# nv-nguyen/gigapose

Hardware: NVIDIA H100
Metric: detections/sec (224x224 crops, 162-template bank) (higher is better)
Workload: dtype f32 (a1, a4, a6: bf16 hi/lo split x3 on tensor cores with fp32 accumulate = fp32-faithful; a5, a7-a9: fp32)

## Files before the change

gigapose_b200/csrc/common.cuh:

```cuda
#pragma once
#include <cuda_runtime.h>
#include <cuda.h>
#include <stdint.h>
#include <cstdio>

namespace gp {

__device__ __forceinline__ uint32_t smem_u32(const void* p) {
  return static_cast<uint32_t>(__cvta_generic_to_shared(p));
}

__device__ __forceinline__ bool elect_one() {
  uint32_t pred = 0;
  asm volatile(
      "{\n\t.reg .pred P;\n\t"
      "elect.sync _|P, 0xffffffff;\n\t"
      "selp.b32 %0, 1, 0, P;\n\t}"
      : "=r"(pred));
  return pred != 0;
}

__device__ __forceinline__ void mbar_init(uint64_t* bar, uint32_t count) {
  asm volatile("mbarrier.init.shared::cta.b64 [%0], %1;" ::"r"(smem_u32(bar)), "r"(count) : "memory");
}
__device__ __forceinline__ void fence_barrier_init() {
  asm volatile("fence.mbarrier_init.release.cluster;" ::: "memory");
}
__device__ __forceinline__ void fence_proxy_async() {
  asm volatile("fence.proxy.async.shared::cta;" ::: "memory");
}
__device__ __forceinline__ void mbar_arrive_expect_tx(uint64_t* bar, uint32_t bytes) {
  asm volatile("mbarrier.arrive.expect_tx.shared::cta.b64 _, [%0], %1;" ::"r"(smem_u32(bar)), "r"(bytes) : "memory");
}
__device__ __forceinline__ void mbar_arrive(uint64_t* bar) {
  asm volatile("mbarrier.arrive.shared::cta.b64 _, [%0];" ::"r"(smem_u32(bar)) : "memory");
}
__device__ __forceinline__ bool mbar_try_wait(uint64_t* bar, uint32_t parity) {
  uint32_t ok;
  asm volatile(
      "{\n\t.reg .pred P;\n\t"
      "mbarrier.try_wait.parity.shared::cta.b64 P, [%1], %2;\n\t"
      "selp.b32 %0, 1, 0, P;\n\t}"
      : "=r"(ok)
      : "r"(smem_u32(bar)), "r"(parity)
      : "memory");
  return ok != 0;
}
__device__ __forceinline__ void mbar_wait(uint64_t* bar, uint32_t parity) {
  uint32_t spins = 0;
  while (!mbar_try_wait(bar, parity)) {
    if (++spins > (1u << 26)) __trap();
  }
}

__device__ __forceinline__ void tma_prefetch_desc(const CUtensorMap* map) {
  asm volatile("prefetch.tensormap [%0];" ::"l"(reinterpret_cast<uint64_t>(map)) : "memory");
}
__device__ __forceinline__ void tma_load_2d(void* smem_dst, const CUtensorMap* map, uint64_t* bar, int32_t c0, int32_t c1) {
  asm volatile(
      "cp.async.bulk.tensor.2d.shared::cluster.global.mbarrier::complete_tx::bytes [%0], [%1, {%3, %4}], [%2];"
      ::"r"(smem_u32(smem_dst)), "l"(reinterpret_cast<uint64_t>(map)), "r"(smem_u32(bar)), "r"(c0), "r"(c1)
      : "memory");
}
__device__ __forceinline__ void tma_load_4d(void* smem_dst, const CUtensorMap* map, uint64_t* bar, int32_t c0, int32_t c1,
                                            int32_t c2, int32_t c3) {
  asm volatile(
      "cp.async.bulk.tensor.4d.shared::cluster.global.mbarrier::complete_tx::bytes [%0], [%1, {%3, %4, %5, %6}], [%2];"
      ::"r"(smem_u32(smem_dst)), "l"(reinterpret_cast<uint64_t>(map)), "r"(smem_u32(bar)), "r"(c0), "r"(c1), "r"(c2), "r"(c3)
      : "memory");
}
constexpr uint64_t kEvictFirst = 0x12F0000000000000ull;
constexpr uint64_t kEvictLast = 0x14F0000000000000ull;
__device__ __forceinline__ void tma_load_2d_hint(void* smem_dst, const CUtensorMap* map, uint64_t* bar, int32_t c0,
                                                 int32_t c1, uint64_t hint) {
  asm volatile(
      "cp.async.bulk.tensor.2d.shared::cluster.global.mbarrier::complete_tx::bytes.L2::cache_hint"
      " [%0], [%1, {%3, %4}], [%2], %5;"
      ::"r"(smem_u32(smem_dst)), "l"(reinterpret_cast<uint64_t>(map)), "r"(smem_u32(bar)), "r"(c0), "r"(c1), "l"(hint)
      : "memory");
}

template <int kRowBytes>
__device__ __forceinline__ uint64_t wgmma_desc_kmajor(uint32_t smem_addr) {
  static_assert(kRowBytes == 128 || kRowBytes == 64 || kRowBytes == 32, "swizzle span");
  constexpr uint64_t layout = kRowBytes == 128 ? 1 : (kRowBytes == 64 ? 2 : 3);
  constexpr uint64_t sbo = (8 * kRowBytes) >> 4;
  uint64_t d = 0;
  d |= static_cast<uint64_t>((smem_addr >> 4) & 0x3FFF);
  d |= 1ull << 16;
  d |= sbo << 32;
  d |= layout << 62;
  return d;
}

__device__ __forceinline__ uint64_t wgmma_desc_mnmajor_sw128(uint32_t smem_addr) {
  uint64_t d = 0;
  d |= static_cast<uint64_t>((smem_addr >> 4) & 0x3FFF);
  d |= 1ull << 16;
  d |= static_cast<uint64_t>(1024 >> 4) << 32;
  d |= 1ull << 62;
  return d;
}

__device__ __forceinline__ void pdl_trigger() { asm volatile("griddepcontrol.launch_dependents;" ::: "memory"); }
__device__ __forceinline__ void pdl_wait() { asm volatile("griddepcontrol.wait;" ::: "memory"); }

__device__ __forceinline__ void named_barrier_sync(uint32_t id, uint32_t nthreads) {
  asm volatile("bar.sync %0, %1;" ::"r"(id), "r"(nthreads) : "memory");
}

template <uint32_t kRegs>
__device__ __forceinline__ void setmaxnreg_dec() { asm volatile("setmaxnreg.dec.sync.aligned.u32 %0;" ::"n"(kRegs)); }
template <uint32_t kRegs>
__device__ __forceinline__ void setmaxnreg_inc() { asm volatile("setmaxnreg.inc.sync.aligned.u32 %0;" ::"n"(kRegs)); }

}
```

gigapose_b200/csrc/vit_attention_tc.cu:

```cuda
#include "gigapose_kernels.h"
#include "common.cuh"
#include "wgmma.cuh"
#include <cuda_bf16.h>

namespace gp {

namespace {

constexpr int kTok = 257, kDim = 1024, kHeads = 16, kHd = 64;
constexpr int kKeys = 272;
constexpr int kRow = 128;
constexpr int kKVPlane = kKeys * kRow;
constexpr int kQPlane = 256 * kRow;
constexpr int kQTiles = 4;
constexpr int kMmaWarps = 8;
constexpr int kThreads = (kMmaWarps + 1) * 32;

struct __align__(8) AttnTail {
  uint64_t qk_full, v_full;
};
constexpr int kSmem = 1024 + 4 * kKVPlane + 2 * kQPlane + sizeof(AttnTail);

__device__ __forceinline__ void split_pair(float a, float b, uint32_t& hi, uint32_t& lo) {
  asm("cvt.rn.bf16x2.f32 %0, %1, %2;" : "=r"(hi) : "f"(b), "f"(a));
  const float ra = a - __uint_as_float(hi << 16), rb = b - __uint_as_float(hi & 0xffff0000u);
  asm("cvt.rn.bf16x2.f32 %0, %1, %2;" : "=r"(lo) : "f"(rb), "f"(ra));
}
__device__ __forceinline__ float ex2_approx(float x) {
  float y;
  asm("ex2.approx.ftz.f32 %0, %1;" : "=f"(y) : "f"(x));
  return y;
}
constexpr float kExpScale = 0.125f * 1.4426950408889634f;
__device__ __forceinline__ float2 ld_pair_sw128(const uint8_t* hi, const uint8_t* lo, int row, int col) {
  const uint32_t off = (uint32_t)row * 128u + ((((uint32_t)col >> 3) ^ ((uint32_t)row & 7u)) << 4) + (((uint32_t)col & 7u) << 1);
  const uint32_t h = *reinterpret_cast<const uint32_t*>(hi + off);
  const uint32_t l = lo ? *reinterpret_cast<const uint32_t*>(lo + off) : 0u;
  return make_float2(__uint_as_float(h << 16) + __uint_as_float(l << 16),
                     __uint_as_float(h & 0xffff0000u) + __uint_as_float(l & 0xffff0000u));
}

}

__device__ long long g_attn_stamp[32];
#define STAMP(i) do { if (blockIdx.x == 0) g_attn_stamp[i] = clock64(); } while (0)

template <int kPasses>
__global__ void __launch_bounds__(kThreads, 1)
attention_tc_kernel(const __grid_constant__ CUtensorMap tm_hi_128, const __grid_constant__ CUtensorMap tm_lo_128,
                    const __grid_constant__ CUtensorMap tm_hi_16, const __grid_constant__ CUtensorMap tm_lo_16,
                    const __nv_bfloat16* __restrict__ qkv_hi, const __nv_bfloat16* __restrict__ qkv_lo,
                    __nv_bfloat16* __restrict__ out_hi, __nv_bfloat16* __restrict__ out_lo, int crop_stride) {
  constexpr int passes = kPasses;
  constexpr int np = passes == 3 ? 2 : 1;
  extern __shared__ uint8_t smem_raw[];
  pdl_trigger();
  uint8_t* smem = smem_raw + ((1024u - (smem_u32(smem_raw) & 1023u)) & 1023u);
  uint8_t* sK[2] = {smem, smem + kKVPlane};
  uint8_t* sV[2] = {smem + 2 * kKVPlane, smem + 3 * kKVPlane};
  uint8_t* sQ[2] = {smem + 4 * kKVPlane, smem + 4 * kKVPlane + kQPlane};
  AttnTail& tail = *reinterpret_cast<AttnTail*>(smem + 4 * kKVPlane + 2 * kQPlane);
  const int warp = threadIdx.x >> 5, lane = threadIdx.x & 31;
  const int item = blockIdx.x;
  const int img = item / kHeads, head = item % kHeads;
  const int row0 = img * kTok;
  const int rq = ((0 * crop_stride + img) * kHeads + head) * kTok;
  const int rk = ((1 * crop_stride + img) * kHeads + head) * kTok;
  const int rv = ((2 * crop_stride + img) * kHeads + head) * kTok;

  if (threadIdx.x == 0) {
    mbar_init(&tail.qk_full, 1);
    mbar_init(&tail.v_full, 1);
    fence_barrier_init();
  }
  __syncthreads();
  pdl_wait();
  if (threadIdx.x == 0) STAMP(0);

  if (warp == kMmaWarps) {
    if (lane == 0) {
      tma_prefetch_desc(&tm_hi_128); tma_prefetch_desc(&tm_hi_16);
      if (np == 2) { tma_prefetch_desc(&tm_lo_128); tma_prefetch_desc(&tm_lo_16); }
      mbar_arrive_expect_tx(&tail.qk_full, (uint32_t)(np * (kQPlane + kKVPlane)));
      for (int pl = 0; pl < np; ++pl) {
        const CUtensorMap* m128 = pl ? &tm_lo_128 : &tm_hi_128;
        const CUtensorMap* m16 = pl ? &tm_lo_16 : &tm_hi_16;
        tma_load_2d(sQ[pl], m128, &tail.qk_full, 0, rq);
        tma_load_2d(sQ[pl] + 128 * kRow, m128, &tail.qk_full, 0, rq + 128);
        tma_load_2d(sK[pl], m128, &tail.qk_full, 0, rk);
        tma_load_2d(sK[pl] + 128 * kRow, m128, &tail.qk_full, 0, rk + 128);
        tma_load_2d(sK[pl] + 256 * kRow, m16, &tail.qk_full, 0, rk + 256);
      }
      mbar_arrive_expect_tx(&tail.v_full, (uint32_t)(np * kKVPlane));
      for (int pl = 0; pl < np; ++pl) {
        const CUtensorMap* m128 = pl ? &tm_lo_128 : &tm_hi_128;
        const CUtensorMap* m16 = pl ? &tm_lo_16 : &tm_hi_16;
        tma_load_2d(sV[pl], m128, &tail.v_full, 0, rv);
        tma_load_2d(sV[pl] + 128 * kRow, m128, &tail.v_full, 0, rv + 128);
        tma_load_2d(sV[pl] + 256 * kRow, m16, &tail.v_full, 0, rv + 256);
      }
    }
    __syncwarp();
    __shared__ float s_p[kKeys];
    __shared__ float s_q[kHd];
    {
    const size_t qoff = (size_t)(rq + 256) * kHd + 2 * lane;
    const uint32_t qh = *reinterpret_cast<const uint32_t*>(qkv_hi + qoff);
    const uint32_t ql = passes == 3 ? *reinterpret_cast<const uint32_t*>(qkv_lo + qoff) : 0u;
    s_q[2 * lane] = __uint_as_float(qh << 16) + __uint_as_float(ql << 16);
    s_q[2 * lane + 1] = __uint_as_float(qh & 0xffff0000u) + __uint_as_float(ql & 0xffff0000u);
    __syncwarp();
    mbar_wait(&tail.qk_full, 0);
    const uint8_t* klo = passes == 3 ? sK[1] : nullptr;
    const uint8_t* vlo = passes == 3 ? sV[1] : nullptr;
    float sj[9];
    float mx = -INFINITY;
#pragma unroll
    for (int i = 0; i < 9; ++i) {
      const int key = lane + 32 * i;
      float acc = 0.f;
      if (key < kTok) {
#pragma unroll
        for (int ch = 0; ch < 8; ++ch) {
          const uint32_t off = (uint32_t)key * 128u + (((uint32_t)ch ^ ((uint32_t)key & 7u)) << 4);
          const uint4 h4 = *reinterpret_cast<const uint4*>(sK[0] + off);
          const uint4 l4 = klo ? *reinterpret_cast<const uint4*>(klo + off) : make_uint4(0, 0, 0, 0);
          const uint32_t hw[4] = {h4.x, h4.y, h4.z, h4.w}, lw[4] = {l4.x, l4.y, l4.z, l4.w};
#pragma unroll
          for (int w = 0; w < 4; ++w) {
            const float k0 = __uint_as_float(hw[w] << 16) + __uint_as_float(lw[w] << 16);
            const float k1 = __uint_as_float(hw[w] & 0xffff0000u) + __uint_as_float(lw[w] & 0xffff0000u);
            acc = fmaf(s_q[ch * 8 + 2 * w], k0, acc);
            acc = fmaf(s_q[ch * 8 + 2 * w + 1], k1, acc);
          }
        }
      }
      sj[i] = key < kTok ? acc : -INFINITY;
      mx = fmaxf(mx, sj[i]);
    }
#pragma unroll
    for (int off = 16; off > 0; off >>= 1) mx = fmaxf(mx, __shfl_xor_sync(0xffffffffu, mx, off));
    float sum = 0.f;
#pragma unroll
    for (int i = 0; i < 9; ++i) {
      const int key = lane + 32 * i;
      const float pj = key < kTok ? ex2_approx((sj[i] - mx) * kExpScale) : 0.f;
      sum += pj;
      if (key < kKeys) s_p[key] = pj;
    }
#pragma unroll
    for (int off = 16; off > 0; off >>= 1) sum += __shfl_xor_sync(0xffffffffu, sum, off);
    __syncwarp();
    mbar_wait(&tail.v_full, 0);
    float o0[4] = {0.f, 0.f, 0.f, 0.f}, o1[4] = {0.f, 0.f, 0.f, 0.f};
#pragma unroll 8
    for (int key = 0; key < 256; ++key) {
      const float2 vv = ld_pair_sw128(sV[0], vlo, key, 2 * lane);
      const float pj = s_p[key];
      o0[key & 3] = fmaf(pj, vv.x, o0[key & 3]);
      o1[key & 3] = fmaf(pj, vv.y, o1[key & 3]);
    }
    {
      const float2 vv = ld_pair_sw128(sV[0], vlo, 256, 2 * lane);
      o0[0] = fmaf(s_p[256], vv.x, o0[0]);
      o1[0] = fmaf(s_p[256], vv.y, o1[0]);
    }
    const float o0s = (o0[0] + o0[1]) + (o0[2] + o0[3]), o1s = (o1[0] + o1[1]) + (o1[2] + o1[3]);
    const float inv = 1.0f / sum;
    uint32_t h, l;
    split_pair(o0s * inv, o1s * inv, h, l);
    const size_t oo = (size_t)(row0 + 256) * kDim + head * kHd + 2 * lane;
    *reinterpret_cast<uint32_t*>(out_hi + oo) = h;
    *reinterpret_cast<uint32_t*>(out_lo + oo) = l;
    }
  } else {
    const int wg = warp >> 2, wl = warp & 3;
    const uint32_t kh = smem_u32(sK[0]), kl = smem_u32(sK[1]), vh = smem_u32(sV[0]), vl = smem_u32(sV[1]);
    mbar_wait(&tail.qk_full, 0);
    if (threadIdx.x == 0) STAMP(1);
    for (int qt = wg; qt < kQTiles; qt += 2) {
      const uint32_t qh = smem_u32(sQ[0] + qt * 64 * kRow), ql = smem_u32(sQ[1] + qt * 64 * kRow);
      float s[128], st[8];
      acc_fence(s); acc_fence(st);
      wgmma_fence();
#pragma unroll
      for (int pass = 0; pass < passes; ++pass) {
        const uint32_t a = pass == 2 ? ql : qh, b = pass == 1 ? kl : kh;
#pragma unroll
        for (int k16 = 0; k16 < 4; ++k16) {
          const uint32_t acc = (pass | k16) != 0 ? 1u : 0u;
          const uint64_t da = wgmma_desc_kmajor<kRow>(a + k16 * 32);
          wgmma_ss_n256_bf16(s, da, wgmma_desc_kmajor<kRow>(b + k16 * 32), acc);
          wgmma_ss_n16_bf16(st, da, wgmma_desc_kmajor<kRow>(b + 256 * kRow + k16 * 32), acc);
        }
      }
      wgmma_commit();
      wgmma_wait<0>();
      acc_fence(s); acc_fence(st);
      const bool key256 = (lane & 3) == 0;
#pragma unroll
      for (int i = 0; i < 8; ++i) if (!(key256 && (i & 1) == 0 && i < 4)) st[i] = -INFINITY;
      float mx0 = fmaxf(st[0], st[1]), mx1 = fmaxf(st[2], st[3]);
#pragma unroll
      for (int j = 0; j < 32; ++j) {
        mx0 = fmaxf(mx0, fmaxf(s[4 * j], s[4 * j + 1]));
        mx1 = fmaxf(mx1, fmaxf(s[4 * j + 2], s[4 * j + 3]));
      }
#pragma unroll
      for (int off = 1; off <= 2; off <<= 1) {
        mx0 = fmaxf(mx0, __shfl_xor_sync(0xffffffffu, mx0, off));
        mx1 = fmaxf(mx1, __shfl_xor_sync(0xffffffffu, mx1, off));
      }
      float sum0 = 0.f, sum1 = 0.f;
      uint32_t ph[68], pl[68];
#pragma unroll
      for (int j = 0; j < 34; ++j) {
        const float x0 = j < 32 ? s[4 * j] : st[4 * (j - 32)], x1 = j < 32 ? s[4 * j + 1] : st[4 * (j - 32) + 1];
        const float x2 = j < 32 ? s[4 * j + 2] : st[4 * (j - 32) + 2], x3 = j < 32 ? s[4 * j + 3] : st[4 * (j - 32) + 3];
        const float p0 = ex2_approx((x0 - mx0) * kExpScale), p1 = ex2_approx((x1 - mx0) * kExpScale);
        const float p2 = ex2_approx((x2 - mx1) * kExpScale), p3 = ex2_approx((x3 - mx1) * kExpScale);
        sum0 += p0 + p1;
        sum1 += p2 + p3;
        const int c = j >> 1, h = (j & 1) * 2;
        split_pair(p0, p1, ph[4 * c + h], pl[4 * c + h]);
        split_pair(p2, p3, ph[4 * c + h + 1], pl[4 * c + h + 1]);
      }
#pragma unroll
      for (int off = 1; off <= 2; off <<= 1) {
        sum0 += __shfl_xor_sync(0xffffffffu, sum0, off);
        sum1 += __shfl_xor_sync(0xffffffffu, sum1, off);
      }
      if (qt == wg) mbar_wait(&tail.v_full, 0);
      float o[32];
      acc_fence(o);
      wgmma_fence();
#pragma unroll
      for (int c = 0; c < kKeys / 16; ++c) {
        const uint32_t ah[4] = {ph[4 * c], ph[4 * c + 1], ph[4 * c + 2], ph[4 * c + 3]};
        const uint64_t dvh = wgmma_desc_mnmajor_sw128(vh + c * 16 * kRow);
        wgmma_rs_n64_bf16_tb(o, ah, dvh, c != 0 ? 1u : 0u);
        if (passes == 3) {
          const uint32_t al[4] = {pl[4 * c], pl[4 * c + 1], pl[4 * c + 2], pl[4 * c + 3]};
          wgmma_rs_n64_bf16_tb(o, ah, wgmma_desc_mnmajor_sw128(vl + c * 16 * kRow), 1u);
          wgmma_rs_n64_bf16_tb(o, al, dvh, 1u);
        }
      }
      wgmma_commit();
      wgmma_wait<0>();
      acc_fence(o);
      const float inv0 = 1.0f / sum0, inv1 = 1.0f / sum1;
      const int tok0 = qt * 64 + wl * 16 + (lane >> 2);
      const size_t o0 = (size_t)(row0 + tok0) * kDim + head * kHd + 2 * (lane & 3);
      const size_t o1 = o0 + (size_t)8 * kDim;
#pragma unroll
      for (int j = 0; j < 8; ++j) {
        uint32_t h, l;
        split_pair(o[4 * j] * inv0, o[4 * j + 1] * inv0, h, l);
        *reinterpret_cast<uint32_t*>(out_hi + o0 + 8 * j) = h;
        *reinterpret_cast<uint32_t*>(out_lo + o0 + 8 * j) = l;
        split_pair(o[4 * j + 2] * inv1, o[4 * j + 3] * inv1, h, l);
        *reinterpret_cast<uint32_t*>(out_hi + o1 + 8 * j) = h;
        *reinterpret_cast<uint32_t*>(out_lo + o1 + 8 * j) = l;
      }
    }
    if (lane == 0 && wl == 0) STAMP(2 + wg);
  }
}

cudaError_t read_attention_stamps(long long* host32) {
  return cudaMemcpyFromSymbol(host32, g_attn_stamp, sizeof(long long) * 32);
}

cudaError_t launch_attention_tc(const CUtensorMap& hi128, const CUtensorMap& lo128, const CUtensorMap& hi16,
                                const CUtensorMap& lo16, const uint16_t* qkv_hi, const uint16_t* qkv_lo, uint16_t* out_hi,
                                uint16_t* out_lo, int b, int crop_stride, int passes, cudaStream_t s) {
  static bool configured = false;
  if (!configured) {
    cudaError_t e = cudaFuncSetAttribute(attention_tc_kernel<3>, cudaFuncAttributeMaxDynamicSharedMemorySize, kSmem);
    if (e == cudaSuccess) e = cudaFuncSetAttribute(attention_tc_kernel<1>, cudaFuncAttributeMaxDynamicSharedMemorySize, kSmem);
    if (e != cudaSuccess) return e;
    configured = true;
  }
  if (b <= 0) return cudaSuccess;
  const int items = b * kHeads;
  const dim3 grid(items);
  auto qh = reinterpret_cast<const __nv_bfloat16*>(qkv_hi), ql = reinterpret_cast<const __nv_bfloat16*>(qkv_lo);
  auto oh = reinterpret_cast<__nv_bfloat16*>(out_hi), ol = reinterpret_cast<__nv_bfloat16*>(out_lo);
  if (passes == 3)
    return launch_ex(attention_tc_kernel<3>, grid, dim3(kThreads), kSmem, s, 1, true, hi128, lo128, hi16, lo16, qh, ql, oh, ol, crop_stride);
  return launch_ex(attention_tc_kernel<1>, grid, dim3(kThreads), kSmem, s, 1, true, hi128, lo128, hi16, lo16, qh, ql, oh, ol, crop_stride);
}

}
```

Baseline: 802.5.

## Make attention kernel persistent with warp-specialized producer and pingpong consumer groups

```diff
diff --git a/gigapose_b200/csrc/common.cuh b/gigapose_b200/csrc/common.cuh
--- a/gigapose_b200/csrc/common.cuh
+++ b/gigapose_b200/csrc/common.cuh
@@ -108,6 +108,9 @@
 __device__ __forceinline__ void named_barrier_sync(uint32_t id, uint32_t nthreads) {
   asm volatile("bar.sync %0, %1;" ::"r"(id), "r"(nthreads) : "memory");
 }
+__device__ __forceinline__ void named_barrier_arrive(uint32_t id, uint32_t nthreads) {
+  asm volatile("bar.arrive %0, %1;" ::"r"(id), "r"(nthreads) : "memory");
+}
 
 template <uint32_t kRegs>
 __device__ __forceinline__ void setmaxnreg_dec() { asm volatile("setmaxnreg.dec.sync.aligned.u32 %0;" ::"n"(kRegs)); }
diff --git a/gigapose_b200/csrc/vit_attention_tc.cu b/gigapose_b200/csrc/vit_attention_tc.cu
--- a/gigapose_b200/csrc/vit_attention_tc.cu
+++ b/gigapose_b200/csrc/vit_attention_tc.cu
@@ -2,6 +2,7 @@
 #include "common.cuh"
 #include "wgmma.cuh"
 #include <cuda_bf16.h>
+#include <algorithm>
 
 namespace gp {
 
@@ -13,13 +14,29 @@
 constexpr int kKVPlane = kKeys * kRow;
 constexpr int kQPlane = 256 * kRow;
 constexpr int kQTiles = 4;
-constexpr int kMmaWarps = 8;
-constexpr int kThreads = (kMmaWarps + 1) * 32;
+constexpr int kConsumerWarps = 8;
+constexpr int kThreads = 128 + kConsumerWarps * 32;
+constexpr int kProducerRegs = 40, kConsumerRegs = 232;
+static_assert(128 * kProducerRegs + kConsumerWarps * 32 * kConsumerRegs <= 65536, "register file");
+constexpr int kKReaders = kConsumerWarps + 3;
+constexpr int kVReaders = kConsumerWarps + 2;
+constexpr uint32_t kTurnBar = 1;
+constexpr uint32_t kTokBar = 3;
 
 struct __align__(8) AttnTail {
-  uint64_t qk_full, v_full;
+  uint64_t qa_full, k_full, qb_full, v_full;
+  uint64_t qa_empty, k_empty, v_empty;
 };
 constexpr int kSmem = 1024 + 4 * kKVPlane + 2 * kQPlane + sizeof(AttnTail);
+
+struct ItemRows {
+  int head, row0, rq, rk, rv;
+};
+__device__ __forceinline__ ItemRows item_rows(int item, int crop_stride) {
+  const int img = item / kHeads, head = item % kHeads;
+  return {head, img * kTok, ((0 * crop_stride + img) * kHeads + head) * kTok, ((1 * crop_stride + img) * kHeads + head) * kTok,
+          ((2 * crop_stride + img) * kHeads + head) * kTok};
+}
 
 __device__ __forceinline__ void split_pair(float a, float b, uint32_t& hi, uint32_t& lo) {
   asm("cvt.rn.bf16x2.f32 %0, %1, %2;" : "=r"(hi) : "f"(b), "f"(a));
@@ -42,6 +59,7 @@
 
 }
 
+constexpr int kStampItems = 10;
 __device__ long long g_attn_stamp[32];
 #define STAMP(i) do { if (blockIdx.x == 0) g_attn_stamp[i] = clock64(); } while (0)
 
@@ -50,7 +68,7 @@
 attention_tc_kernel(const __grid_constant__ CUtensorMap tm_hi_128, const __grid_constant__ CUtensorMap tm_lo_128,
                     const __grid_constant__ CUtensorMap tm_hi_16, const __grid_constant__ CUtensorMap tm_lo_16,
                     const __nv_bfloat16* __restrict__ qkv_hi, const __nv_bfloat16* __restrict__ qkv_lo,
-                    __nv_bfloat16* __restrict__ out_hi, __nv_bfloat16* __restrict__ out_lo, int crop_stride) {
+                    __nv_bfloat16* __restrict__ out_hi, __nv_bfloat16* __restrict__ out_lo, int crop_stride, int items) {
   constexpr int passes = kPasses;
   constexpr int np = passes == 3 ? 2 : 1;
   extern __shared__ uint8_t smem_raw[];
@@ -61,209 +79,265 @@
   uint8_t* sQ[2] = {smem + 4 * kKVPlane, smem + 4 * kKVPlane + kQPlane};
   AttnTail& tail = *reinterpret_cast<AttnTail*>(smem + 4 * kKVPlane + 2 * kQPlane);
   const int warp = threadIdx.x >> 5, lane = threadIdx.x & 31;
-  const int item = blockIdx.x;
-  const int img = item / kHeads, head = item % kHeads;
-  const int row0 = img * kTok;
-  const int rq = ((0 * crop_stride + img) * kHeads + head) * kTok;
-  const int rk = ((1 * crop_stride + img) * kHeads + head) * kTok;
-  const int rv = ((2 * crop_stride + img) * kHeads + head) * kTok;
 
   if (threadIdx.x == 0) {
-    mbar_init(&tail.qk_full, 1);
+    mbar_init(&tail.qa_full, 1);
+    mbar_init(&tail.k_full, 1);
+    mbar_init(&tail.qb_full, 1);
     mbar_init(&tail.v_full, 1);
+    mbar_init(&tail.qa_empty, kConsumerWarps);
+    mbar_init(&tail.k_empty, kKReaders);
+    mbar_init(&tail.v_empty, kVReaders);
     fence_barrier_init();
+  }
+  if (warp == 0 && lane == 0) {
+    tma_prefetch_desc(&tm_hi_128); tma_prefetch_desc(&tm_hi_16);
+    if (np == 2) { tma_prefetch_desc(&tm_lo_128); tma_prefetch_desc(&tm_lo_16); }
   }
   __syncthreads();
   pdl_wait();
   if (threadIdx.x == 0) STAMP(0);
 
-  if (warp == kMmaWarps) {
-    if (lane == 0) {
-      tma_prefetch_desc(&tm_hi_128); tma_prefetch_desc(&tm_hi_16);
-      if (np == 2) { tma_prefetch_desc(&tm_lo_128); tma_prefetch_desc(&tm_lo_16); }
-      mbar_arrive_expect_tx(&tail.qk_full, (uint32_t)(np * (kQPlane + kKVPlane)));
-      for (int pl = 0; pl < np; ++pl) {
-        const CUtensorMap* m128 = pl ? &tm_lo_128 : &tm_hi_128;
-        const CUtensorMap* m16 = pl ? &tm_lo_16 : &tm_hi_16;
-        tma_load_2d(sQ[pl], m128, &tail.qk_full, 0, rq);
-        tma_load_2d(sQ[pl] + 128 * kRow, m128, &tail.qk_full, 0, rq + 128);
-        tma_load_2d(sK[pl], m128, &tail.qk_full, 0, rk);
-        tma_load_2d(sK[pl] + 128 * kRow, m128, &tail.qk_full, 0, rk + 128);
-        tma_load_2d(sK[pl] + 256 * kRow, m16, &tail.qk_full, 0, rk + 256);
+  if (warp < 4) {
+    setmaxnreg_dec<kProducerRegs>();
+    if (warp == 0 && lane == 0) {
+      uint32_t it = 0;
+      for (int item = blockIdx.x; item < items; item += gridDim.x, ++it) {
+        const ItemRows r = item_rows(item, crop_stride);
+        if (it > 0) mbar_wait(&tail.qa_empty, (it - 1) & 1u);
+        mbar_arrive_expect_tx(&tail.qa_full, (uint32_t)(np * kQPlane / 2));
+        for (int pl = 0; pl < np; ++pl) tma_load_2d(sQ[pl], pl ? &tm_lo_128 : &tm_hi_128, &tail.qa_full, 0, r.rq);
+        if (it > 0) mbar_wait(&tail.k_empty, (it - 1) & 1u);
+        mbar_arrive_expect_tx(&tail.k_full, (uint32_t)(np * kKVPlane));
+        for (int pl = 0; pl < np; ++pl) {
+          const CUtensorMap* m128 = pl ? &tm_lo_128 : &tm_hi_128;
+          const CUtensorMap* m16 = pl ? &tm_lo_16 : &tm_hi_16;
+          tma_load_2d(sK[pl], m128, &tail.k_full, 0, r.rk);
+          tma_load_2d(sK[pl] + 128 * kRow, m128, &tail.k_full, 0, r.rk + 128);
+          tma_load_2d(sK[pl] + 256 * kRow, m16, &tail.k_full, 0, r.rk + 256);
+        }
+        mbar_arrive_expect_tx(&tail.qb_full, (uint32_t)(np * kQPlane / 2));
+        for (int pl = 0; pl < np; ++pl)
+          tma_load_2d(sQ[pl] + 128 * kRow, pl ? &tm_lo_128 : &tm_hi_128, &tail.qb_full, 0, r.rq + 128);
+        if (it > 0) mbar_wait(&tail.v_empty, (it - 1) & 1u);
+        mbar_arrive_expect_tx(&tail.v_full, (uint32_t)(np * kKVPlane));
+        for (int pl = 0; pl < np; ++pl) {
+          const CUtensorMap* m128 = pl ? &tm_lo_128 : &tm_hi_128;
+          const CUtensorMap* m16 = pl ? &tm_lo_16 : &tm_hi_16;
+          tma_load_2d(sV[pl], m128, &tail.v_full, 0, r.rv);
+          tma_load_2d(sV[pl] + 128 * kRow, m128, &tail.v_full, 0, r.rv + 128);
+          tma_load_2d(sV[pl] + 256 * kRow, m16, &tail.v_full, 0, r.rv + 256);
+        }
       }
-      mbar_arrive_expect_tx(&tail.v_full, (uint32_t)(np * kKVPlane));
-      for (int pl = 0; pl < np; ++pl) {
-        const CUtensorMap* m128 = pl ? &tm_lo_128 : &tm_hi_128;
-        const CUtensorMap* m16 = pl ? &tm_lo_16 : &tm_hi_16;
-        tma_load_2d(sV[pl], m128, &tail.v_full, 0, rv);
-        tma_load_2d(sV[pl] + 128 * kRow, m128, &tail.v_full, 0, rv + 128);
-        tma_load_2d(sV[pl] + 256 * kRow, m16, &tail.v_full, 0, rv + 256);
+    } else if (warp >= 1) {
+      __shared__ float s_p[kKeys];
+      __shared__ float s_q[kHd];
+      __shared__ float s_o23[kHd];
+      const int tt = threadIdx.x - 32;
+      const uint8_t* klo = passes == 3 ? sK[1] : nullptr;
+      const uint8_t* vlo = passes == 3 ? sV[1] : nullptr;
+      uint32_t it = 0;
+      for (int item = blockIdx.x; item < items; item += gridDim.x, ++it) {
+        if (warp == 1) {
+          const ItemRows r = item_rows(item, crop_stride);
+          const size_t qoff = (size_t)(r.rq + 256) * kHd + 2 * lane;
+          const uint32_t qh = *reinterpret_cast<const uint32_t*>(qkv_hi + qoff);
+          const uint32_t ql = passes == 3 ? *reinterpret_cast<const uint32_t*>(qkv_lo + qoff) : 0u;
+          s_q[2 * lane] = __uint_as_float(qh << 16) + __uint_as_float(ql << 16);
+          s_q[2 * lane + 1] = __uint_as_float(qh & 0xffff0000u) + __uint_as_float(ql & 0xffff0000u);
+        }
+        named_barrier_sync(kTokBar, 96);
+        mbar_wait(&tail.k_full, it & 1u);
+#pragma unroll 1
+        for (int key = tt; key < kKeys; key += 96) {
+          float acc = 0.f;
+          if (key < kTok) {
+#pragma unroll 1
+            for (int ch = 0; ch < 8; ++ch) {
+              const uint32_t off = (uint32_t)key * 128u + (((uint32_t)ch ^ ((uint32_t)key & 7u)) << 4);
+              const uint4 h4 = *reinterpret_cast<const uint4*>(sK[0] + off);
+              const uint4 l4 = klo ? *reinterpret_cast<const uint4*>(klo + off) : make_uint4(0, 0, 0, 0);
+              const uint32_t hw[4] = {h4.x, h4.y, h4.z, h4.w}, lw[4] = {l4.x, l4.y, l4.z, l4.w};
+#pragma unroll
+              for (int w = 0; w < 4; ++w) {
+                const float k0 = __uint_as_float(hw[w] << 16) + __uint_as_float(lw[w] << 16);
+                const float k1 = __uint_as_float(hw[w] & 0xffff0000u) + __uint_as_float(lw[w] & 0xffff0000u);
+                acc = fmaf(s_q[ch * 8 + 2 * w], k0, acc);
+                acc = fmaf(s_q[ch * 8 + 2 * w + 1], k1, acc);
+              }
+            }
+          }
+          s_p[key] = key < kTok ? acc : -INFINITY;
+        }
+        __syncwarp();
+        if (lane == 0) mbar_arrive(&tail.k_empty);
+        named_barrier_sync(kTokBar, 96);
+        float sum = 0.f;
+        if (warp == 1) {
+          float mx = -INFINITY;
+#pragma unroll
+          for (int i = 0; i < 9; ++i) {
+            const int key = lane + 32 * i;
+            mx = fmaxf(mx, key < kTok ? s_p[key] : -INFINITY);
+          }
+#pragma unroll
+          for (int off = 16; off > 0; off >>= 1) mx = fmaxf(mx, __shfl_xor_sync(0xffffffffu, mx, off));
+#pragma unroll
+          for (int i = 0; i < 9; ++i) {
+            const int key = lane + 32 * i;
+            const float pj = key < kTok ? ex2_approx((s_p[key] - mx) * kExpScale) : 0.f;
+            sum += pj;
+            if (key < kKeys) s_p[key] = pj;
+          }
+#pragma unroll
+          for (int off = 16; off > 0; off >>= 1) sum += __shfl_xor_sync(0xffffffffu, sum, off);
+        }
+        named_barrier_sync(kTokBar, 96);
+        if (warp == 3) continue;
+        mbar_wait(&tail.v_full, it & 1u);
+        const int k0 = warp == 1 ? 0 : 2;
+        float o0[2] = {0.f, 0.f}, o1[2] = {0.f, 0.f};
+#pragma unroll 4
+        for (int kb = 0; kb < 256; kb += 4) {
+#pragma unroll
+          for (int c = 0; c < 2; ++c) {
+            const int key = kb + k0 + c;
+            const float2 vv = ld_pair_sw128(sV[0], vlo, key, 2 * lane);
+            const float pj = s_p[key];
+            o0[c] = fmaf(pj, vv.x, o0[c]);
+            o1[c] = fmaf(pj, vv.y, o1[c]);
+          }
+        }
+        if (warp == 1) {
+          const float2 vv = ld_pair_sw128(sV[0], vlo, 256, 2 * lane);
+          o0[0] = fmaf(s_p[256], vv.x, o0[0]);
+          o1[0] = fmaf(s_p[256], vv.y, o1[0]);
+        }
+        __syncwarp();
+        if (lane == 0) mbar_arrive(&tail.v_empty);
+        if (warp == 2) {
+          s_o23[2 * lane] = o0[0] + o0[1];
+          s_o23[2 * lane + 1] = o1[0] + o1[1];
+          named_barrier_arrive(kTokBar + 1, 64);
+        } else {
+          named_barrier_sync(kTokBar + 1, 64);
+          const float o0s = (o0[0] + o0[1]) + s_o23[2 * lane], o1s = (o1[0] + o1[1]) + s_o23[2 * lane + 1];
+          const float inv = 1.0f / sum;
+          uint32_t h, l;
+          split_pair(o0s * inv, o1s * inv, h, l);
+          const ItemRows r = item_rows(item, crop_stride);
+          const size_t oo = (size_t)(r.row0 + 256) * kDim + r.head * kHd + 2 * lane;
+          *reinterpret_cast<uint32_t*>(out_hi + oo) = h;
+          *reinterpret_cast<uint32_t*>(out_lo + oo) = l;
+        }
       }
     }
-    __syncwarp();
-    __shared__ float s_p[kKeys];
-    __shared__ float s_q[kHd];
-    {
-    const size_t qoff = (size_t)(rq + 256) * kHd + 2 * lane;
-    const uint32_t qh = *reinterpret_cast<const uint32_t*>(qkv_hi + qoff);
-    const uint32_t ql = passes == 3 ? *reinterpret_cast<const uint32_t*>(qkv_lo + qoff) : 0u;
-    s_q[2 * lane] = __uint_as_float(qh << 16) + __uint_as_float(ql << 16);
-    s_q[2 * lane + 1] = __uint_as_float(qh & 0xffff0000u) + __uint_as_float(ql & 0xffff0000u);
-    __syncwarp();
-    mbar_wait(&tail.qk_full, 0);
-    const uint8_t* klo = passes == 3 ? sK[1] : nullptr;
-    const uint8_t* vlo = passes == 3 ? sV[1] : nullptr;
-    float sj[9];
-    float mx = -INFINITY;
-#pragma unroll
-    for (int i = 0; i < 9; ++i) {
-      const int key = lane + 32 * i;
-      float acc = 0.f;
-      if (key < kTok) {
-#pragma unroll
-        for (int ch = 0; ch < 8; ++ch) {
-          const uint32_t off = (uint32_t)key * 128u + (((uint32_t)ch ^ ((uint32_t)key & 7u)) << 4);
-          const uint4 h4 = *reinterpret_cast<const uint4*>(sK[0] + off);
-          const uint4 l4 = klo ? *reinterpret_cast<const uint4*>(klo + off) : make_uint4(0, 0, 0, 0);
-          const uint32_t hw[4] = {h4.x, h4.y, h4.z, h4.w}, lw[4] = {l4.x, l4.y, l4.z, l4.w};
-#pragma unroll
-          for (int w = 0; w < 4; ++w) {
-            const float k0 = __uint_as_float(hw[w] << 16) + __uint_as_float(lw[w] << 16);
-            const float k1 = __uint_as_float(hw[w] & 0xffff0000u) + __uint_as_float(lw[w] & 0xffff0000u);
-            acc = fmaf(s_q[ch * 8 + 2 * w], k0, acc);
-            acc = fmaf(s_q[ch * 8 + 2 * w + 1], k1, acc);
-          }
+  } else {
+    setmaxnreg_inc<kConsumerRegs>();
+    const int wg = (warp - 4) >> 2, wl = warp & 3;
+    const uint32_t kh = smem_u32(sK[0]), kl = smem_u32(sK[1]), vh = smem_u32(sV[0]), vl = smem_u32(sV[1]);
+    if (wg == 1) named_barrier_arrive(kTurnBar + 0, 256);
+    uint32_t it = 0;
+    for (int item = blockIdx.x; item < items; item += gridDim.x, ++it) {
+      const ItemRows r = item_rows(item, crop_stride);
+      const bool last_item = item + (int)gridDim.x >= items;
+      mbar_wait(&tail.qa_full, it & 1u);
+      mbar_wait(&tail.k_full, it & 1u);
+      if (threadIdx.x == 128 && it < kStampItems) STAMP(1 + 3 * it);
+      for (int qt = wg; qt < kQTiles; qt += 2) {
+        const uint32_t qh = smem_u32(sQ[0] + qt * 64 * kRow), ql = smem_u32(sQ[1] + qt * 64 * kRow);
+        if (qt >= 2) mbar_wait(&tail.qb_full, it & 1u);
+        float s[128], st[8];
+        acc_fence(s); acc_fence(st);
+        named_barrier_sync(kTurnBar + wg, 256);
+        wgmma_fence();
+#pragma unroll
+        for (int pass = 0; pass < passes; ++pass) {
+          const uint32_t a = pass == 2 ? ql : qh, b = pass == 1 ? kl : kh;
+#pragma unroll
+          for (int k16 = 0; k16 < 4; ++k16) {
+            const uint32_t acc = (pass | k16) != 0 ? 1u : 0u;
+            const uint64_t da = wgmma_desc_kmajor<kRow>(a + k16 * 32);
+            wgmma_ss_n256_bf16(s, da, wgmma_desc_kmajor<kRow>(b + k16 * 32), acc);
+            wgmma_ss_n16_bf16(st, da, wgmma_desc_kmajor<kRow>(b + 256 * kRow + k16 * 32), acc);
+          }
+        }
+        wgmma_commit();
+        named_barrier_arrive(kTurnBar + (wg ^ 1), 256);
+        wgmma_wait<0>();
+        acc_fence(s); acc_fence(st);
+        if (lane == 0) mbar_arrive(qt < 2 ? &tail.qa_empty : &tail.k_empty);
+        const bool key256 = (lane & 3) == 0;
+#pragma unroll
+        for (int i = 0; i < 8; ++i) if (!(key256 && (i & 1) == 0 && i < 4)) st[i] = -INFINITY;
+        float mx0 = fmaxf(st[0], st[1]), mx1 = fmaxf(st[2], st[3]);
+#pragma unroll
+        for (int j = 0; j < 32; ++j) {
+          mx0 = fmaxf(mx0, fmaxf(s[4 * j], s[4 * j + 1]));
+          mx1 = fmaxf(mx1, fmaxf(s[4 * j + 2], s[4 * j + 3]));
+        }
+#pragma unroll
+        for (int off = 1; off <= 2; off <<= 1) {
+          mx0 = fmaxf(mx0, __shfl_xor_sync(0xffffffffu, mx0, off));
+          mx1 = fmaxf(mx1, __shfl_xor_sync(0xffffffffu, mx1, off));
+        }
+        float sum0 = 0.f, sum1 = 0.f;
+        uint32_t ph[68], pl[68];
+#pragma unroll
+        for (int j = 0; j < 34; ++j) {
+          const float x0 = j < 32 ? s[4 * j] : st[4 * (j - 32)], x1 = j < 32 ? s[4 * j + 1] : st[4 * (j - 32) + 1];
+          const float x2 = j < 32 ? s[4 * j + 2] : st[4 * (j - 32) + 2], x3 = j < 32 ? s[4 * j + 3] : st[4 * (j - 32) + 3];
+          const float p0 = ex2_approx((x0 - mx0) * kExpScale), p1 = ex2_approx((x1 - mx0) * kExpScale);
+          const float p2 = ex2_approx((x2 - mx1) * kExpScale), p3 = ex2_approx((x3 - mx1) * kExpScale);
+          sum0 += p0 + p1;
+          sum1 += p2 + p3;
+          const int c = j >> 1, h = (j & 1) * 2;
+          split_pair(p0, p1, ph[4 * c + h], pl[4 * c + h]);
+          split_pair(p2, p3, ph[4 * c + h + 1], pl[4 * c + h + 1]);
+        }
+#pragma unroll
+        for (int off = 1; off <= 2; off <<= 1) {
+          sum0 += __shfl_xor_sync(0xffffffffu, sum0, off);
+          sum1 += __shfl_xor_sync(0xffffffffu, sum1, off);
+        }
+        if (qt == wg) mbar_wait(&tail.v_full, it & 1u);
+        float o[32];
+        acc_fence(o);
+        named_barrier_sync(kTurnBar + wg, 256);
+        wgmma_fence();
+#pragma unroll
+        for (int c = 0; c < kKeys / 16; ++c) {
+          const uint32_t ah[4] = {ph[4 * c], ph[4 * c + 1], ph[4 * c + 2], ph[4 * c + 3]};
+          const uint64_t dvh = wgmma_desc_mnmajor_sw128(vh + c * 16 * kRow);
+          wgmma_rs_n64_bf16_tb(o, ah, dvh, c != 0 ? 1u : 0u);
+          if (passes == 3) {
+            const uint32_t al[4] = {pl[4 * c], pl[4 * c + 1], pl[4 * c + 2], pl[4 * c + 3]};
+            wgmma_rs_n64_bf16_tb(o, ah, wgmma_desc_mnmajor_sw128(vl + c * 16 * kRow), 1u);
+            wgmma_rs_n64_bf16_tb(o, al, dvh, 1u);
+          }
+        }
+        wgmma_commit();
+        if (!(wg == 1 && qt >= 2 && last_item)) named_barrier_arrive(kTurnBar + (wg ^ 1), 256);
+        wgmma_wait<0>();
+        acc_fence(o);
+        if (qt >= 2 && lane == 0) mbar_arrive(&tail.v_empty);
+        const float inv0 = 1.0f / sum0, inv1 = 1.0f / sum1;
+        const int tok0 = qt * 64 + wl * 16 + (lane >> 2);
+        const size_t o0 = (size_t)(r.row0 + tok0) * kDim + r.head * kHd + 2 * (lane & 3);
+        const size_t o1 = o0 + (size_t)8 * kDim;
+#pragma unroll
+        for (int j = 0; j < 8; ++j) {
+          uint32_t h, l;
+          split_pair(o[4 * j] * inv0, o[4 * j + 1] * inv0, h, l);
+          *reinterpret_cast<uint32_t*>(out_hi + o0 + 8 * j) = h;
+          *reinterpret_cast<uint32_t*>(out_lo + o0 + 8 * j) = l;
+          split_pair(o[4 * j + 2] * inv1, o[4 * j + 3] * inv1, h, l);
+          *reinterpret_cast<uint32_t*>(out_hi + o1 + 8 * j) = h;
+          *reinterpret_cast<uint32_t*>(out_lo + o1 + 8 * j) = l;
         }
       }
-      sj[i] = key < kTok ? acc : -INFINITY;
-      mx = fmaxf(mx, sj[i]);
+      if (lane == 0 && wl == 0 && it < kStampItems) STAMP(2 + 3 * it + wg);
     }
-#pragma unroll
-    for (int off = 16; off > 0; off >>= 1) mx = fmaxf(mx, __shfl_xor_sync(0xffffffffu, mx, off));
-    float sum = 0.f;
-#pragma unroll
-    for (int i = 0; i < 9; ++i) {
-      const int key = lane + 32 * i;
-      const float pj = key < kTok ? ex2_approx((sj[i] - mx) * kExpScale) : 0.f;
-      sum += pj;
-      if (key < kKeys) s_p[key] = pj;
-    }
-#pragma unroll
-    for (int off = 16; off > 0; off >>= 1) sum += __shfl_xor_sync(0xffffffffu, sum, off);
-    __syncwarp();
-    mbar_wait(&tail.v_full, 0);
-    float o0[4] = {0.f, 0.f, 0.f, 0.f}, o1[4] = {0.f, 0.f, 0.f, 0.f};
-#pragma unroll 8
-    for (int key = 0; key < 256; ++key) {
-      const float2 vv = ld_pair_sw128(sV[0], vlo, key, 2 * lane);
-      const float pj = s_p[key];
-      o0[key & 3] = fmaf(pj, vv.x, o0[key & 3]);
-      o1[key & 3] = fmaf(pj, vv.y, o1[key & 3]);
-    }
-    {
-      const float2 vv = ld_pair_sw128(sV[0], vlo, 256, 2 * lane);
-      o0[0] = fmaf(s_p[256], vv.x, o0[0]);
-      o1[0] = fmaf(s_p[256], vv.y, o1[0]);
-    }
-    const float o0s = (o0[0] + o0[1]) + (o0[2] + o0[3]), o1s = (o1[0] + o1[1]) + (o1[2] + o1[3]);
-    const float inv = 1.0f / sum;
-    uint32_t h, l;
-    split_pair(o0s * inv, o1s * inv, h, l);
-    const size_t oo = (size_t)(row0 + 256) * kDim + head * kHd + 2 * lane;
-    *reinterpret_cast<uint32_t*>(out_hi + oo) = h;
-    *reinterpret_cast<uint32_t*>(out_lo + oo) = l;
-    }
-  } else {
-    const int wg = warp >> 2, wl = warp & 3;
-    const uint32_t kh = smem_u32(sK[0]), kl = smem_u32(sK[1]), vh = smem_u32(sV[0]), vl = smem_u32(sV[1]);
-    mbar_wait(&tail.qk_full, 0);
-    if (threadIdx.x == 0) STAMP(1);
-    for (int qt = wg; qt < kQTiles; qt += 2) {
-      const uint32_t qh = smem_u32(sQ[0] + qt * 64 * kRow), ql = smem_u32(sQ[1] + qt * 64 * kRow);
-      float s[128], st[8];
-      acc_fence(s); acc_fence(st);
-      wgmma_fence();
-#pragma unroll
-      for (int pass = 0; pass < passes; ++pass) {
-        const uint32_t a = pass == 2 ? ql : qh, b = pass == 1 ? kl : kh;
-#pragma unroll
-        for (int k16 = 0; k16 < 4; ++k16) {
-          const uint32_t acc = (pass | k16) != 0 ? 1u : 0u;
-          const uint64_t da = wgmma_desc_kmajor<kRow>(a + k16 * 32);
-          wgmma_ss_n256_bf16(s, da, wgmma_desc_kmajor<kRow>(b + k16 * 32), acc);
-          wgmma_ss_n16_bf16(st, da, wgmma_desc_kmajor<kRow>(b + 256 * kRow + k16 * 32), acc);
-        }
-      }
-      wgmma_commit();
-      wgmma_wait<0>();
-      acc_fence(s); acc_fence(st);
-      const bool key256 = (lane & 3) == 0;
-#pragma unroll
-      for (int i = 0; i < 8; ++i) if (!(key256 && (i & 1) == 0 && i < 4)) st[i] = -INFINITY;
-      float mx0 = fmaxf(st[0], st[1]), mx1 = fmaxf(st[2], st[3]);
-#pragma unroll
-      for (int j = 0; j < 32; ++j) {
-        mx0 = fmaxf(mx0, fmaxf(s[4 * j], s[4 * j + 1]));
-        mx1 = fmaxf(mx1, fmaxf(s[4 * j + 2], s[4 * j + 3]));
-      }
-#pragma unroll
-      for (int off = 1; off <= 2; off <<= 1) {
-        mx0 = fmaxf(mx0, __shfl_xor_sync(0xffffffffu, mx0, off));
-        mx1 = fmaxf(mx1, __shfl_xor_sync(0xffffffffu, mx1, off));
-      }
-      float sum0 = 0.f, sum1 = 0.f;
-      uint32_t ph[68], pl[68];
-#pragma unroll
-      for (int j = 0; j < 34; ++j) {
-        const float x0 = j < 32 ? s[4 * j] : st[4 * (j - 32)], x1 = j < 32 ? s[4 * j + 1] : st[4 * (j - 32) + 1];
-        const float x2 = j < 32 ? s[4 * j + 2] : st[4 * (j - 32) + 2], x3 = j < 32 ? s[4 * j + 3] : st[4 * (j - 32) + 3];
-        const float p0 = ex2_approx((x0 - mx0) * kExpScale), p1 = ex2_approx((x1 - mx0) * kExpScale);
-        const float p2 = ex2_approx((x2 - mx1) * kExpScale), p3 = ex2_approx((x3 - mx1) * kExpScale);
-        sum0 += p0 + p1;
-        sum1 += p2 + p3;
-        const int c = j >> 1, h = (j & 1) * 2;
-        split_pair(p0, p1, ph[4 * c + h], pl[4 * c + h]);
-        split_pair(p2, p3, ph[4 * c + h + 1], pl[4 * c + h + 1]);
-      }
-#pragma unroll
-      for (int off = 1; off <= 2; off <<= 1) {
-        sum0 += __shfl_xor_sync(0xffffffffu, sum0, off);
-        sum1 += __shfl_xor_sync(0xffffffffu, sum1, off);
-      }
-      if (qt == wg) mbar_wait(&tail.v_full, 0);
-      float o[32];
-      acc_fence(o);
-      wgmma_fence();
-#pragma unroll
-      for (int c = 0; c < kKeys / 16; ++c) {
-        const uint32_t ah[4] = {ph[4 * c], ph[4 * c + 1], ph[4 * c + 2], ph[4 * c + 3]};
-        const uint64_t dvh = wgmma_desc_mnmajor_sw128(vh + c * 16 * kRow);
-        wgmma_rs_n64_bf16_tb(o, ah, dvh, c != 0 ? 1u : 0u);
-        if (passes == 3) {
-          const uint32_t al[4] = {pl[4 * c], pl[4 * c + 1], pl[4 * c + 2], pl[4 * c + 3]};
-          wgmma_rs_n64_bf16_tb(o, ah, wgmma_desc_mnmajor_sw128(vl + c * 16 * kRow), 1u);
-          wgmma_rs_n64_bf16_tb(o, al, dvh, 1u);
-        }
-      }
-      wgmma_commit();
-      wgmma_wait<0>();
-      acc_fence(o);
-      const float inv0 = 1.0f / sum0, inv1 = 1.0f / sum1;
-      const int tok0 = qt * 64 + wl * 16 + (lane >> 2);
-      const size_t o0 = (size_t)(row0 + tok0) * kDim + head * kHd + 2 * (lane & 3);
-      const size_t o1 = o0 + (size_t)8 * kDim;
-#pragma unroll
-      for (int j = 0; j < 8; ++j) {
-        uint32_t h, l;
-        split_pair(o[4 * j] * inv0, o[4 * j + 1] * inv0, h, l);
-        *reinterpret_cast<uint32_t*>(out_hi + o0 + 8 * j) = h;
-        *reinterpret_cast<uint32_t*>(out_lo + o0 + 8 * j) = l;
-        split_pair(o[4 * j + 2] * inv1, o[4 * j + 3] * inv1, h, l);
-        *reinterpret_cast<uint32_t*>(out_hi + o1 + 8 * j) = h;
-        *reinterpret_cast<uint32_t*>(out_lo + o1 + 8 * j) = l;
-      }
-    }
-    if (lane == 0 && wl == 0) STAMP(2 + wg);
   }
 }
 
@@ -282,13 +356,19 @@
     configured = true;
   }
   if (b <= 0) return cudaSuccess;
+  int dev = 0, sms = 0;
+  cudaError_t e = cudaGetDevice(&dev);
+  if (e == cudaSuccess) e = cudaDeviceGetAttribute(&sms, cudaDevAttrMultiProcessorCount, dev);
+  if (e != cudaSuccess) return e;
   const int items = b * kHeads;
-  const dim3 grid(items);
+  const dim3 grid(std::min(items, sms));
   auto qh = reinterpret_cast<const __nv_bfloat16*>(qkv_hi), ql = reinterpret_cast<const __nv_bfloat16*>(qkv_lo);
   auto oh = reinterpret_cast<__nv_bfloat16*>(out_hi), ol = reinterpret_cast<__nv_bfloat16*>(out_lo);
   if (passes == 3)
-    return launch_ex(attention_tc_kernel<3>, grid, dim3(kThreads), kSmem, s, 1, true, hi128, lo128, hi16, lo16, qh, ql, oh, ol, crop_stride);
-  return launch_ex(attention_tc_kernel<1>, grid, dim3(kThreads), kSmem, s, 1, true, hi128, lo128, hi16, lo16, qh, ql, oh, ol, crop_stride);
-}
-
-}
+    return launch_ex(attention_tc_kernel<3>, grid, dim3(kThreads), kSmem, s, 1, true, hi128, lo128, hi16, lo16, qh, ql, oh, ol,
+                     crop_stride, items);
+  return launch_ex(attention_tc_kernel<1>, grid, dim3(kThreads), kSmem, s, 1, true, hi128, lo128, hi16, lo16, qh, ql, oh, ol,
+                   crop_stride, items);
+}
+
+}
```

Result: no change. 808.5, median of 6 (+0.8%).
